# NICTA/revrand

Hardware: AMD Instinct MI355X
Metric: feature-rows/sec (Phi + PhiT Phi + PhiT y) at N=10M D=32 F=4096 (higher is better)
Workload: dtype f32; 1 GPU; RandomRBF nbases=2048 (F=4096), D=32, N=10000000 f32, features + MFMA Gram, rows sharded over 1 GPU(s); rows_per_gpu=10000000, device=(gfx950:sramecc+:xnack-), gram_engine=f32

## Files before the change

### revrand_amd/csrc/rr_mfma_tile.h

```cpp
#pragma once
#include <hip/hip_runtime.h>
#include <cstdint>
#include <cstdlib>

typedef float floatx16 __attribute__((ext_vector_type(16)));
typedef __attribute__((address_space(1))) const void *gptr_t;
typedef __attribute__((address_space(3))) void *lptr_t;

constexpr int GR_TC = 256;
constexpr int GR_KB = 32;
constexpr int GR_LD = 512;
constexpr int GR_THREADS = 512;

typedef float float2v __attribute__((ext_vector_type(2)));

typedef __amdgpu_buffer_rsrc_t rr_rsrc_t;
typedef unsigned rr_u4_t __attribute__((ext_vector_type(4)));
__device__ __forceinline__ rr_rsrc_t rr_make_rsrc(const void *base, unsigned bytes) {
    const uint64_t a = (uint64_t)base;
    const unsigned lo = (unsigned)__builtin_amdgcn_readfirstlane((unsigned)a), hi = (unsigned)__builtin_amdgcn_readfirstlane((unsigned)(a >> 32));
    return __builtin_amdgcn_make_buffer_rsrc((void *)(((uint64_t)hi << 32) | (uint64_t)lo), 0, (int)__builtin_amdgcn_readfirstlane(bytes),
                                             0x00020000);
}

__device__ __forceinline__ void rr_dma_kblock(const float *pa, int64_t lda, const float *pb, int64_t ldb, float *buf, int wave,
                                              unsigned voff) {
    const rr_rsrc_t ra = rr_make_rsrc(pa, 0x7fffffffu), rb = rr_make_rsrc(pb, 0x7fffffffu);
    const unsigned lda4 = (unsigned)lda * 4u, ldb4 = (unsigned)ldb * 4u;
#pragma unroll
    for (int k = 0; k < 4; ++k) {
        const int lr = 4 * wave + k;
        float *dst = buf + lr * GR_LD;
        __builtin_amdgcn_raw_ptr_buffer_load_lds(ra, (lptr_t)dst, 16, voff, (unsigned)lr * lda4, 0, 0);
        __builtin_amdgcn_raw_ptr_buffer_load_lds(rb, (lptr_t)(dst + GR_TC), 16, voff, (unsigned)lr * ldb4, 0, 0);
    }
}
__device__ __forceinline__ int rr_dma_slot(int wave, int spread = 2) {
    return spread == 2 ? (wave < 4 ? wave : ((wave + 2) & 3)) : spread == 1 ? (wave >> 2) : 0;
}
inline int rr_dma_spread_env() {
    const char *e = getenv("RR_DMA_SPREAD");
    return e ? atoi(e) : 2;
}

template <int O0, int O1>
__device__ __forceinline__ float2v lds_read2st64(unsigned addr) {
    float2v r;
    asm volatile("ds_read2st64_b32 %0, %1 offset0:%2 offset1:%3" : "=v"(r) : "v"(addr), "i"(O0), "i"(O1));
    return r;
}
__device__ __forceinline__ void lds_wait() { asm volatile("s_waitcnt lgkmcnt(0)" ::: "memory"); }

struct KOps2 {
    float2v a[4], b[2];
    template <int P>
    __device__ __forceinline__ void load(const unsigned (&abase)[4], const unsigned (&bbase)[2]) {
#pragma unroll
        for (int i = 0; i < 4; ++i) a[i] = lds_read2st64<32 * P, 32 * P + 16>(abase[i]);
#pragma unroll
        for (int j = 0; j < 2; ++j) b[j] = lds_read2st64<32 * P, 32 * P + 16>(bbase[j]);
    }
};

template <int FIRST, int LAST>
__device__ __forceinline__ void gram_mfma(const KOps2 &o, floatx16 (&acc)[4][2]) {
#pragma unroll
    for (int q = FIRST; q < LAST; ++q)
        acc[(q >> 1) & 3][q & 1] = __builtin_amdgcn_mfma_f32_32x32x2f32(o.a[(q >> 1) & 3][q >> 3], o.b[q & 1][q >> 3],
                                                                        acc[(q >> 1) & 3][q & 1], 0, 0, 0);
}

#define RR_PAIR(P, CUR, NXT)                                   \
    lds_wait();                                                \
    __builtin_amdgcn_sched_barrier(0);                         \
    gram_mfma<0, 1>(CUR, acc);                                 \
    __builtin_amdgcn_sched_barrier(0);                         \
    if ((P) + 1 < 8) NXT.template load<((P) + 1) & 7>(abase, bbase); \
    __builtin_amdgcn_sched_barrier(0);                         \
    gram_mfma<1, 16>(CUR, acc);                                \
    __builtin_amdgcn_sched_barrier(0);

__device__ __forceinline__ void gram_consume(unsigned cur, floatx16 (&acc)[4][2], unsigned aoff, unsigned boff) {
    unsigned abase[4], bbase[2];
#pragma unroll
    for (int i = 0; i < 4; ++i) abase[i] = cur + aoff + i * 128;
#pragma unroll
    for (int j = 0; j < 2; ++j) bbase[j] = cur + boff + j * 128;
    KOps2 o0, o1;
    o0.load<0>(abase, bbase);
    RR_PAIR(0, o0, o1) RR_PAIR(1, o1, o0) RR_PAIR(2, o0, o1) RR_PAIR(3, o1, o0)
    RR_PAIR(4, o0, o1) RR_PAIR(5, o1, o0) RR_PAIR(6, o0, o1) RR_PAIR(7, o1, o0)
}

template <typename DMA>
__device__ __forceinline__ void gram_consume_staggered(unsigned cur, floatx16 (&acc)[4][2], unsigned aoff, unsigned boff, int slot,
                                                       DMA dma) {
    unsigned abase[4], bbase[2];
#pragma unroll
    for (int i = 0; i < 4; ++i) abase[i] = cur + aoff + i * 128;
#pragma unroll
    for (int j = 0; j < 2; ++j) bbase[j] = cur + boff + j * 128;
    KOps2 o0, o1;
    if (slot == 0) dma();
    o0.load<0>(abase, bbase);
    RR_PAIR(0, o0, o1)
    if (slot == 1) dma();
    RR_PAIR(1, o1, o0)
    if (slot == 2) dma();
    RR_PAIR(2, o0, o1)
    if (slot == 3) dma();
    RR_PAIR(3, o1, o0)
    RR_PAIR(4, o0, o1) RR_PAIR(5, o1, o0) RR_PAIR(6, o0, o1) RR_PAIR(7, o1, o0)
}
#undef RR_PAIR
```

### revrand_amd/csrc/rr_rff.hip

```cpp
#include "rr_syrk_args.h"
#include <algorithm>
#include <map>
#include <mutex>
#include <type_traits>




__device__ __forceinline__ void sincos_rev(float t, float &s, float &c) {
    const float f = t - __builtin_rintf(t);
    s = __builtin_amdgcn_sinf(f);
    c = __builtin_amdgcn_cosf(f);
}

__device__ __forceinline__ void sincos_rev(double t, double &s, double &c) { rr_sincos_rev_f64(t, s, c); }
typedef double doublex4 __attribute__((ext_vector_type(4)));

template <int DMAX, bool GUARD, typename TX, typename TC>
__device__ __forceinline__ TC project_row(const TX *__restrict__ xr, int d, const TC (&w)[DMAX]) {
    TC z = 0;
#pragma unroll
    for (int i = 0; i < DMAX; ++i) {
        if (!GUARD || i < d) z = fma((TC)xr[i], w[i], z);
    }
// ... 483 lines not shown
    for (int64_t tl = tile0 + wave; tl < tile1; tl += 4) {
        const int64_t r0 = tl * 16;
        double a[KS];
        {
            const int64_t ra = r0 + j;
            const TX *src = X + (ra < N ? ra : 0) * ldx + g * KS;
#pragma unroll
            for (int t = 0; t < KS; ++t) a[t] = (double)src[t];
            if (ra >= N) {
#pragma unroll
                for (int t = 0; t < KS; ++t) a[t] = 0.0;
            }
        }
        const int64_t d0 = N - r0;
        const int lim = (int)(d0 > 16 ? 16 : (d0 < 0 ? 0 : d0));
        double yv[4];
        if (HAS_Y) {
            const int64_t ry = r0 + j;
            double yt = (double)y[ry < N ? ry : N - 1];
            yt = ry < N ? yt : 0.0;
            const int lo = __double2loint(yt), hi = __double2hiint(yt);
#pragma unroll
            for (int e = 0; e < 4; ++e) {
                const int srcl = 4 * (g + 4 * e);
                yv[e] = __hiloint2double(__builtin_amdgcn_ds_bpermute(srcl, hi), __builtin_amdgcn_ds_bpermute(srcl, lo));
            }
        }
        const char *tile_c = (const char *)(P + r0 * ldp + c0);
        const char *tile_s = tile_c + (int64_t)n * (int64_t)sizeof(TO);
        constexpr unsigned ES = sizeof(TO);
        const unsigned lane_off = ES * ((unsigned)g * (unsigned)ldp + (unsigned)j);
#pragma unroll
        for (int cb = 0; cb < CB; ++cb) {
            doublex4 acc = {0.0, 0.0, 0.0, 0.0};
#pragma unroll
            for (int t = 0; t < KS; ++t) acc = __builtin_amdgcn_mfma_f64_16x16x4f64(a[t], bw[cb][t], acc, 0, 0, 0);
            if (c0 + 16 * cb + j < n) {
#pragma unroll
                for (int e = 0; e < 4; ++e) {
                    const int rr = g + 4 * e;
                    const unsigned off = lane_off + ES * 4u * (unsigned)e * (unsigned)ldp;
                    if constexpr (ES == 8) {
                        double sv, cv;
                        rr_sincos_rev_f64(acc[e], sv, cv);
                        cv = rr < lim ? cv * scale : 0.0;
                        sv = rr < lim ? sv * scale : 0.0;
                        asm volatile("global_store_dwordx2 %0, %1, %2 offset:%3 nt" ::"v"(off), "v"(cv), "s"(tile_c), "i"(128 * cb) : "memory");
                        asm volatile("global_store_dwordx2 %0, %1, %2 offset:%3 nt" ::"v"(off), "v"(sv), "s"(tile_s), "i"(128 * cb) : "memory");
                        if (HAS_Y) {
                            bc[cb] = fma(cv, yv[e], bc[cb]);
                            bs[cb] = fma(sv, yv[e], bs[cb]);
                        }
                    } else {
                        const float fr = (float)(acc[e] - rint(acc[e]));
                        const float fs = (float)scale;
                        float cf = __builtin_amdgcn_cosf(fr), sf = __builtin_amdgcn_sinf(fr);
                        cf = rr < lim ? cf * fs : 0.f;
                        sf = rr < lim ? sf * fs : 0.f;
                        asm volatile("global_store_dword %0, %1, %2 offset:%3" RR_NT_ASM ::"v"(off), "v"(cf), "s"(tile_c), "i"(64 * cb) : "memory");
                        asm volatile("global_store_dword %0, %1, %2 offset:%3" RR_NT_ASM ::"v"(off), "v"(sf), "s"(tile_s), "i"(64 * cb) : "memory");
                        if (HAS_Y) {
                            bc[cb] = fma((double)cf, yv[e], bc[cb]);
                            bs[cb] = fma((double)sf, yv[e], bs[cb]);
                        }
                    }
                }
            }
        }
    }
    if (HAS_Y) {
#pragma unroll
        for (int cb = 0; cb < CB; ++cb) {
#pragma unroll
            for (int m = 16; m < 64; m <<= 1) {
                bc[cb] += __hiloint2double(__shfl_xor(__double2hiint(bc[cb]), m, 64), __shfl_xor(__double2loint(bc[cb]), m, 64));
                bs[cb] += __hiloint2double(__shfl_xor(__double2hiint(bs[cb]), m, 64), __shfl_xor(__double2loint(bs[cb]), m, 64));
            }
            const int col = c0 + 16 * cb + j;
            if (g == 0 && col < n) {
                rr_acc_out(bvec, bdet, (int64_t)blockIdx.y * 4 + wave, col, bc[cb]);
                rr_acc_out(bvec, bdet, (int64_t)blockIdx.y * 4 + wave, n + col, bs[cb]);
            }
        }
    }
}

template <typename TX, typename TO>
static bool rr_features_mfma64_launch(rr_basis *b, const TX *X, const TX *y, int64_t m, int64_t mpad, int64_t ldx, TO *P,
                                      int64_t ldp, double *db, double scale) {
    static const bool disabled = getenv("RR_FEATURES_NO_MFMA64") != nullptr;
    if (disabled || b->large || ((ldx * sizeof(TX)) & 15) != 0 || ((uintptr_t)X & 15) != 0 || b->dpad < 8 || m < 1) return false;
    if ((uint64_t)sizeof(TO) * 20u * (uint64_t)ldp >= (1ull << 32)) return false;
    rr_ctx *c = b->ctx;
    const int64_t ntiles = (mpad + 15) / 16;
#define RR_FM64(DM, CBK)                                                                                            \
    do {                                                                                                            \
        const int cgroups = (b->n + 16 * CBK - 1) / (16 * CBK);                                                     \
        int64_t tpb = 128;                                                                                          \
        while (tpb > 4 && cgroups * ((ntiles + tpb - 1) / tpb) < 8 * (int64_t)c->num_cu) tpb >>= 1;                 \
        if ((ntiles + tpb - 1) / tpb > 65535) tpb = (ntiles + 65534) / 65535;                                       \
        const dim3 grid(cgroups, (unsigned)((ntiles + tpb - 1) / tpb));                                             \
        if (y && c->deterministic) {                                                                                \
            void *part = nullptr;                                                                                   \
            const int64_t nslots = (int64_t)grid.y * 4, F2 = 2 * (int64_t)b->n;                                     \
            if (rr_det_scratch(c, (size_t)nslots * F2 * 8, &part) != RR_OK) return false;                           \
            hipLaunchKernelGGL((rr_rff_features_mfma64_kernel<DM, CBK, true, TX, TO>), grid, dim3(256), 0, c->stream, \
                               X, y, m, mpad, ldx, b->dWs64, b->n, b->npad, P, ldp, (double *)part, scale, (int)tpb, F2); \
            if (rr_det_reduce(c, (const double *)part, nslots, F2, F2, db) != RR_OK) return false;                  \
        } else if (y) hipLaunchKernelGGL((rr_rff_features_mfma64_kernel<DM, CBK, true, TX, TO>), grid, dim3(256), 0, c->stream, \
                                  X, y, m, mpad, ldx, b->dWs64, b->n, b->npad, P, ldp, db, scale, (int)tpb);        \
        else hipLaunchKernelGGL((rr_rff_features_mfma64_kernel<DM, CBK, false, TX, TO>), grid, dim3(256), 0, c->stream, \
                                X, y, m, mpad, ldx, b->dWs64, b->n, b->npad, P, ldp, db, scale, (int)tpb);          \
    } while (0)
    switch (b->dpad) {
        case 8: RR_FM64(8, 4); break;
        case 16: RR_FM64(16, 4); break;
        case 32: RR_FM64(32, 4); break;
        case 64: RR_FM64(64, 2); break;
        case 128: RR_FM64(128, 1); break;
        default: return false;
    }
#undef RR_FM64
    return true;
}

template <typename TC>
__global__ void __launch_bounds__(256) rr_zero_padcols_kernel(TC *P, int64_t rows, int64_t ldp, int F) {
    const int w = (int)ldp - F;
    const int64_t i = (int64_t)blockIdx.x * blockDim.x + threadIdx.x;
    if (w > 0 && i < rows * w) P[(i / w) * ldp + F + (i % w)] = TC(0);
}

__global__ void __launch_bounds__(256) rr_zero_padcols_pb_kernel(uintx4 *Pb, int64_t ksteps, int64_t ldp, int F) {
    const int64_t w = (ldp - F) * 4;
    const int64_t i = (int64_t)blockIdx.x * blockDim.x + threadIdx.x;
    if (w > 0 && i < ksteps * w) Pb[(i / w) * ldp * 4 + (int64_t)F * 4 + (i % w)] = uintx4{0u, 0u, 0u, 0u};
}



__device__ __forceinline__ void syrk_dma_tile(const SyrkArgs &p, float *buf, int64_t kb0, int wave, int lane,
                                              int ca, int cb) {
#pragma unroll
    for (int k = 0; k < 4; ++k) {
        const int lr = 4 * wave + k;
        RR_DEV_ASSERT(kb0 + lr < p.rows && ca + GR_TC <= p.ldp && cb + GR_TC <= p.ldp);
        const float *src = p.P + (kb0 + lr) * p.ldp + 4 * lane;
        float *dst = buf + lr * GR_LD;
        __builtin_amdgcn_global_load_lds((gptr_t)(src + ca), (lptr_t)dst, 16, 0, 0);
        __builtin_amdgcn_global_load_lds((gptr_t)(src + cb), (lptr_t)(dst + GR_TC), 16, 0, 0);
    }
}

template <int MODE>
__device__ __forceinline__ void rr_syrk_f32_body(const SyrkArgs &p, float *lds, const unsigned bid) {
    constexpr bool STAG = (MODE & 1) != 0, BUF = (MODE & 2) != 0;

    const int tid = threadIdx.x;
    const int lane = tid & 63;
    const int wave = __builtin_amdgcn_readfirstlane(tid >> 6);

    int tdx = bid % p.ntiles;
    const int ks = bid / p.ntiles;
    if (p.tile_map) tdx = p.tile_map[tdx];
    int ta = 0;
    const int od = p.offdiag_only;
    while (tdx >= p.nb - ta - od) {
        tdx -= p.nb - ta - od;
        ++ta;
    }
    const int tb = ta + tdx + od;
    const bool diag = (ta == tb);
    const int ca = ta * GR_TC, cb = tb * GR_TC;

    const int64_t row_begin = (int64_t)ks * p.rows_per_split;
    int64_t row_end = row_begin + p.rows_per_split;
    if (row_end > p.rows) row_end = p.rows;

    const int wr = wave >> 2, wc_ = wave & 3;
    const unsigned aoff = 4u * ((lane >> 5) * GR_LD + wr * 128 + (lane & 31));
    const unsigned boff = 4u * ((lane >> 5) * GR_LD + GR_TC + wc_ * 64 + (lane & 31));
    const unsigned lds0 = (unsigned)(size_t)(__attribute__((address_space(3))) float *)lds;
    floatx16 acc[4][2];
#pragma unroll
    for (int i = 0; i < 4; ++i)
#pragma unroll
        for (int j = 0; j < 2; ++j)
#pragma unroll
            for (int e = 0; e < 16; ++e) acc[i][j][e] = 0.f;

    const int64_t nkb = (row_end - row_begin) / GR_KB;
    RR_DEV_ASSERT(p.rows % GR_KB == 0 && p.rows_per_split % GR_KB == 0 && tb < p.nb && p.nb * GR_TC <= p.ldp);
    if (BUF && nkb > 0) {
        const unsigned voff = 16u * lane;
        const float *Pa = p.P + row_begin * p.ldp + ca, *Pb = p.P + row_begin * p.ldp + cb;
        rr_dma_kblock(Pa, p.ldp, Pb, p.ldp, lds, wave, voff);
        __syncthreads();
        for (int64_t kb = 0; kb < nkb; ++kb) {
            const int cbuf = (int)(kb & 1);
            float *nxt = lds + (cbuf ^ 1) * (GR_KB * GR_LD);
            const int64_t ro = (kb + 1) * GR_KB * p.ldp;
            if (STAG) {
                gram_consume_staggered(lds0 + cbuf * (4u * GR_KB * GR_LD), acc, aoff, boff, rr_dma_slot(wave, p.spread), [&]() {
                    if (kb + 1 < nkb) rr_dma_kblock(Pa + ro, p.ldp, Pb + ro, p.ldp, nxt, wave, voff);
                });
            } else {
                if (kb + 1 < nkb) rr_dma_kblock(Pa + ro, p.ldp, Pb + ro, p.ldp, nxt, wave, voff);
                gram_consume(lds0 + cbuf * (4u * GR_KB * GR_LD), acc, aoff, boff);
            }
            __syncthreads();
        }
    } else if (nkb > 0) {
        syrk_dma_tile(p, lds, row_begin, wave, lane, ca, cb);
        __syncthreads();
        for (int64_t kb = 0; kb < nkb; ++kb) {
            const int cbuf = (int)(kb & 1);
            float *nxt = lds + (cbuf ^ 1) * (GR_KB * GR_LD);
            if (STAG) {
                const int slot = (wave < 4) ? wave : ((wave + 2) & 3);
                gram_consume_staggered(lds0 + cbuf * (4u * GR_KB * GR_LD), acc, aoff, boff, slot, [&]() {
                    if (kb + 1 < nkb) syrk_dma_tile(p, nxt, row_begin + (kb + 1) * GR_KB, wave, lane, ca, cb);
                });
                __syncthreads();
                continue;
            }
            if (kb + 1 < nkb && !(p.ablate & 1)) syrk_dma_tile(p, nxt, row_begin + (kb + 1) * GR_KB, wave, lane, ca, cb);
            gram_consume(lds0 + cbuf * (4u * GR_KB * GR_LD), acc, aoff, boff);
            if (!(p.ablate & 2)) __syncthreads();
        }
    }

    if (p.ablate & 4) return;
    const int64_t F = p.F;
    const int hi = lane >> 5;
#pragma unroll
    for (int j = 0; j < 2; ++j) {
        const int64_t gc = cb + wc_ * 64 + j * 32 + (lane & 31);
#pragma unroll
        for (int i = 0; i < 4; ++i) {
#pragma unroll
            for (int e = 0; e < 16; ++e) {
                const int64_t gr = ca + wr * 128 + i * 32 + (e & 3) + 8 * (e >> 2) + 4 * hi;
                if (gr <= gc) rr_syrk_out(p, ks, gr, gc, acc[i][j][e]);
            }
        }
    }
    (void)diag;
    (void)F;
}

#define RR_SYRK_KERNEL(NAME, MODE)                                                       \
    __global__ void __launch_bounds__(GR_THREADS, 2) NAME(const SyrkArgs p) {             \
        __shared__ float lds[2 * GR_KB * GR_LD];                                          \
        rr_syrk_f32_body<MODE>(p, lds, blockIdx.x);                                       \
    }
RR_SYRK_KERNEL(rr_syrk_f32_kernel, 3)
RR_SYRK_KERNEL(rr_syrk_f32_flat_kernel, 0)
RR_SYRK_KERNEL(rr_syrk_f32_flatstag_kernel, 1)
RR_SYRK_KERNEL(rr_syrk_f32_buf_kernel, 2)
#undef RR_SYRK_KERNEL

template <int NI>
struct KOpsR {
    float2v a[NI], b[2];
    template <int P>
    __device__ __forceinline__ void load(const unsigned (&abase)[NI], const unsigned (&bbase)[2]) {
#pragma unroll
        for (int i = 0; i < NI; ++i) a[i] = lds_read2st64<32 * P, 32 * P + 16>(abase[i]);
#pragma unroll
        for (int j = 0; j < 2; ++j) b[j] = lds_read2st64<32 * P, 32 * P + 16>(bbase[j]);
    }
};

template <int NI, int FIRST, int LAST>
__device__ __forceinline__ void gram_mfma_r(const KOpsR<NI> &o, floatx16 (&acc)[NI][2]) {
#pragma unroll
    for (int q = FIRST; q < LAST; ++q) {
        constexpr int dummy = 0;
        (void)dummy;
        const int s_ = q / (2 * NI), r_ = q % (2 * NI);
        acc[r_ >> 1][r_ & 1] = __builtin_amdgcn_mfma_f32_32x32x2f32(o.a[r_ >> 1][s_], o.b[r_ & 1][s_], acc[r_ >> 1][r_ & 1], 0, 0, 0);
    }
}

#define RR_PAIRR(P, CUR, NXT)                                  \
    lds_wait();                                                \
    __builtin_amdgcn_sched_barrier(0);                         \
    gram_mfma_r<NI, 0, 1>(CUR, acc);                           \
    __builtin_amdgcn_sched_barrier(0);                         \
    if ((P) + 1 < 8) NXT.template load<((P) + 1) & 7>(abase, bbase); \
    __builtin_amdgcn_sched_barrier(0);                         \
    gram_mfma_r<NI, 1, 4 * NI>(CUR, acc);                      \
    __builtin_amdgcn_sched_barrier(0);

template <int NI>
__device__ __forceinline__ void syrk_ragged_loop(const SyrkArgs &p, float *lds, int wave, int lane, int ca, int cb,
                                                 int64_t row_begin, int64_t nkb, int ks) {
    const int wr = wave >> 2, wc_ = wave & 3;
    const unsigned aoff = 4u * ((lane >> 5) * GR_LD + wr * 128 + (lane & 31));
    const unsigned boff = 4u * ((lane >> 5) * GR_LD + GR_TC + wc_ * 64 + (lane & 31));
    const unsigned lds0 = (unsigned)(size_t)(__attribute__((address_space(3))) float *)lds;
    constexpr int NA = NI > 0 ? NI : 1;
    floatx16 acc[NA][2];
#pragma unroll
    for (int i = 0; i < NA; ++i)
#pragma unroll
        for (int j = 0; j < 2; ++j)
#pragma unroll
            for (int e = 0; e < 16; ++e) acc[i][j][e] = 0.f;
    if (nkb > 0) {
        syrk_dma_tile(p, lds, row_begin, wave, lane, ca, cb);
        __syncthreads();
        for (int64_t kb = 0; kb < nkb; ++kb) {
            const int cbuf = (int)(kb & 1);
            if (kb + 1 < nkb) syrk_dma_tile(p, lds + (cbuf ^ 1) * (GR_KB * GR_LD), row_begin + (kb + 1) * GR_KB, wave, lane, ca, cb);
            if constexpr (NI > 0) {
                const unsigned cur = lds0 + cbuf * (4u * GR_KB * GR_LD);
                unsigned abase[NI], bbase[2];
#pragma unroll
                for (int i = 0; i < NI; ++i) abase[i] = cur + aoff + i * 128;
#pragma unroll
                for (int j = 0; j < 2; ++j) bbase[j] = cur + boff + j * 128;
                KOpsR<NI> o0, o1;
                o0.template load<0>(abase, bbase);
                RR_PAIRR(0, o0, o1) RR_PAIRR(1, o1, o0) RR_PAIRR(2, o0, o1) RR_PAIRR(3, o1, o0)
                RR_PAIRR(4, o0, o1) RR_PAIRR(5, o1, o0) RR_PAIRR(6, o0, o1) RR_PAIRR(7, o1, o0)
            }
            __syncthreads();
        }
    }
    if constexpr (NI > 0) {
        const int hi = lane >> 5;
#pragma unroll
        for (int j = 0; j < 2; ++j) {
            const int64_t grow = cb + wc_ * 64 + j * 32 + (lane & 31);
#pragma unroll
            for (int i = 0; i < NI; ++i) {
#pragma unroll
                for (int e = 0; e < 16; ++e) {
                    const int64_t gcol = ca + wr * 128 + i * 32 + (e & 3) + 8 * (e >> 2) + 4 * hi;
                    rr_syrk_out(p, ks, grow, gcol, acc[i][j][e]);
                }
            }
        }
    }
}
#undef RR_PAIRR

__global__ void __launch_bounds__(GR_THREADS, 2)
rr_syrk_f32_ragged_kernel(const SyrkArgs p) {
    __shared__ float lds[2 * GR_KB * GR_LD];
    const int lane = threadIdx.x & 63;
    const int wave = __builtin_amdgcn_readfirstlane(threadIdx.x >> 6);
    const int last = p.nb - 1;
    const int ta = blockIdx.x % last;
    const int ks = blockIdx.x / last;
    const int ca = last * GR_TC;
    const int cb = ta * GR_TC;
    const int64_t row_begin = (int64_t)ks * p.rows_per_split;
    int64_t row_end = row_begin + p.rows_per_split;
    if (row_end > p.rows) row_end = p.rows;
    const int64_t nkb = (row_end - row_begin) / GR_KB;
    RR_DEV_ASSERT(p.rows % GR_KB == 0 && p.rows_per_split % GR_KB == 0 && p.nb * GR_TC == p.ldp && p.F > ca);
    const int w = p.F + (p.bcol ? 1 : 0) - ca;
    int ni = (w - (wave >> 2) * 128 + 31) / 32;
    ni = ni < 0 ? 0 : (ni > 4 ? 4 : ni);
    switch (ni) {
        case 0: syrk_ragged_loop<0>(p, lds, wave, lane, ca, cb, row_begin, nkb, ks); break;
        case 1: syrk_ragged_loop<1>(p, lds, wave, lane, ca, cb, row_begin, nkb, ks); break;
        case 2: syrk_ragged_loop<2>(p, lds, wave, lane, ca, cb, row_begin, nkb, ks); break;
        case 3: syrk_ragged_loop<3>(p, lds, wave, lane, ca, cb, row_begin, nkb, ks); break;
        default: syrk_ragged_loop<4>(p, lds, wave, lane, ca, cb, row_begin, nkb, ks); break;
    }
}

__constant__ unsigned char RR_DIAG_I[8][5] = {{0, 0, 0, 0, 0}, {1, 1, 1, 1, 1}, {2, 2, 2, 2, 2}, {3, 3, 3, 3, 3},
                                              {0, 0, 0, 7, 0}, {1, 1, 6, 6, 1}, {2, 5, 5, 5, 2}, {4, 4, 4, 4, 4}};
__constant__ unsigned char RR_DIAG_J[8][5] = {{0, 1, 2, 3, 4}, {1, 2, 3, 4, 5}, {2, 3, 4, 5, 6}, {3, 4, 5, 6, 7},
                                              {5, 6, 7, 7, 5}, {6, 7, 6, 7, 6}, {7, 5, 6, 7, 7}, {4, 5, 6, 7, 4}};

template <int NB>
struct KOpsD {
    float2v a[NB], b[NB];
    template <int P>
    __device__ __forceinline__ void load(const unsigned (&abase)[NB], const unsigned (&bbase)[NB]) {
#pragma unroll
        for (int e = 0; e < NB; ++e) a[e] = lds_read2st64<16 * P, 16 * P + 8>(abase[e]);
#pragma unroll
        for (int e = 0; e < NB; ++e) b[e] = lds_read2st64<16 * P, 16 * P + 8>(bbase[e]);
    }
};

template <int NB, int FIRST, int LAST>
__device__ __forceinline__ void gram_mfma_d(const KOpsD<NB> &o, floatx16 (&acc)[NB]) {
#pragma unroll
    for (int q = FIRST; q < LAST; ++q)
        acc[q % NB] = __builtin_amdgcn_mfma_f32_32x32x2f32(o.a[q % NB][q / NB], o.b[q % NB][q / NB], acc[q % NB], 0, 0, 0);
}

#define RR_PAIRD(P, CUR, NXT)                                  \
    lds_wait();                                                \
    __builtin_amdgcn_sched_barrier(0);                         \
    gram_mfma_d<NB, 0, 1>(CUR, acc);                           \
    __builtin_amdgcn_sched_barrier(0);                         \
    if ((P) + 1 < 8) NXT.template load<((P) + 1) & 7>(abase, bbase); \
    __builtin_amdgcn_sched_barrier(0);                         \
    gram_mfma_d<NB, 1, 2 * NB>(CUR, acc);                      \
    __builtin_amdgcn_sched_barrier(0);

template <int NB>
__device__ __forceinline__ void syrk_diag_body(const SyrkArgs &p, float *lds, int wave, int lane) {
    const int ta = blockIdx.x % p.nb;
    const int ks = blockIdx.x / p.nb;
// ... 1359 lines not shown
            if (d <= 0 || (double)(next() >> 11) / 9007199254740992.0 < exp(-(double)d / temp)) {
                add(x, t1, -1); add(y, t2, -1); add(x, t2, 1); add(y, t1, 1);
                part[t1] = y; part[t2] = x;
                cur += d;
                if (cur < best) { best = cur; best_part = part; }
            }
        }
        part = best_part;
    }
    std::vector<int> fill(nxcd, 0);
    for (int t = 0; t < ntiles; ++t) map[(size_t)fill[part[t]]++ * nxcd + part[t]] = t;
}


int rr_launch_syrk_f32(rr_ctx *c, const float *P, int64_t rows, int64_t ldp, int F, double *dG, hipEvent_t mid,
                       double *bcol = nullptr) {
    if (c->gram_engine != 0) {
        RR_REQUIRE(bcol == nullptr, "gram: the rider column needs the f32 engine");
        RR_REQUIRE(!c->deterministic, "gram: deterministic mode (rr_set_deterministic) needs the f32 engine, not a split 16-bit one");
        return rr_launch_syrk_bf16(c, c->gram_engine, P, nullptr, rows, ldp, F, dG, mid);
    }
    RR_REQUIRE(bcol == nullptr || F < ldp, "gram: no pad column for the rider");
    static const bool small_off = getenv("RR_SYRK_SMALL") != nullptr && atoi(getenv("RR_SYRK_SMALL")) == 0;
    const int64_t big_tiles = (ldp / GR_TC) * (ldp / GR_TC + 1) / 2;
    if (!small_off && ldp <= 1024 && big_tiles * ((rows + 1023) / 1024) < c->num_cu && rows % GS_KB == 0 && !getenv("RR_GRAM_ABLATE")) {
        const int nbs = (int)(ldp / GS_TC), nt = nbs * (nbs + 1) / 2;
        int64_t ns = std::max<int64_t>((2 * c->num_cu + nt - 1) / nt, (rows + 32767) / 32768);
        ns = std::min<int64_t>(ns, std::max<int64_t>(rows / 128, 1));
        const int64_t rps_s = ((rows + ns - 1) / ns + GS_KB - 1) / GS_KB * GS_KB;
        ns = (rows + rps_s - 1) / rps_s;
        SyrkArgs a;
        a.P = P; a.rows = rows; a.ldp = ldp; a.F = F; a.nb = nbs; a.ntiles = nt; a.rows_per_split = rps_s; a.G = dG;
        a.bcol = bcol; a.tile_map = nullptr; a.offdiag_only = 0; a.ablate = 0;
        if (c->deterministic) {
            void *slabs = nullptr;
            int rc = rr_det_scratch(c, (size_t)ns * (size_t)ldp * (size_t)ldp * sizeof(float), &slabs);
            if (rc != RR_OK) return rc;
            a.part = (float *)slabs;
            a.part_stride = ldp * ldp;
        }
        hipLaunchKernelGGL(rr_syrk_f32_small_kernel, dim3((unsigned)(ns * nt)), dim3(GS_THREADS), 0, c->stream, a);
        if (mid) RR_CHECK_HIP(hipEventRecord(mid, c->stream));
        if (a.part)
            hipLaunchKernelGGL(rr_syrk_det_reduce_kernel<float>, dim3((unsigned)((F + 1 + 255) / 256), (unsigned)F), dim3(256), 0,
                               c->stream, a.part, a.part_stride, ldp, F, (int)ns, dG, bcol);
        RR_CHECK_HIP(hipGetLastError());
        return RR_OK;
    }
    const int nb_all = (int)(ldp / GR_TC);
    const int od = (nb_all >= 2 && !getenv("RR_SYRK_NO_DIAG_KERNEL")) ? 1 : 0;
    const int w_last = F + (bcol ? 1 : 0) - GR_TC * (nb_all - 1);
    const int rg = (od && nb_all >= 3 && w_last <= 192 && !getenv("RR_SYRK_NO_RAGGED_KERNEL")) ? 1 : 0;
    const int nb = nb_all - rg;
    const int ntiles = od ? nb * (nb - 1) / 2 : nb * (nb + 1) / 2;
    const int nxcd = 8;
    const bool use_map = (ntiles % nxcd == 0) && !getenv("RR_GRAM_NO_TILE_MAP");
    if (use_map && c->tile_map_nb != nb * 2 + od) {
        std::vector<int> map;
        rr_build_tile_map(nb, od, nxcd, map);
        if (c->tile_map) (void)hipFree(c->tile_map);
        c->tile_map = nullptr;
        RR_CHECK_HIP(hipMalloc((void **)&c->tile_map, map.size() * sizeof(int)));
        RR_CHECK_HIP(hipMemcpy(c->tile_map, map.data(), map.size() * sizeof(int), hipMemcpyHostToDevice));
        c->tile_map_nb = nb * 2 + od;
    }
    const int64_t total_tiles = (int64_t)nb_all * (nb_all + 1) / 2;
    auto gcd64 = [](int64_t x, int64_t y) { while (y) { const int64_t u = x % y; x = y; y = u; } return x; };
    const int64_t min_splits = (rows + 32767) / 32768;
    auto rows_per = [&](int64_t ns) { return ((rows + ns - 1) / ns + GR_KB - 1) / GR_KB * GR_KB; };
    const int64_t unit = ntiles > 0 ? c->num_cu / gcd64(c->num_cu, ntiles) : 1;
    int64_t nsplit = (min_splits + unit - 1) / unit * unit;
    auto floor_rows = [&](int64_t tiles_per_split) {
        return tiles_per_split * ((rows + 1023) / 1024) < c->num_cu ? (int64_t)256 : (int64_t)1024;
    };
    auto small_split = [&](int64_t tiles_per_split) {
        const int64_t fr = floor_rows(tiles_per_split);
        if (fr == 1024) return (rows + 1023) / 1024;
        const int64_t want = (c->num_cu + tiles_per_split - 1) / std::max<int64_t>(tiles_per_split, 1);
        return std::min((rows + fr - 1) / fr, std::max((rows + 1023) / 1024, want));
    };
    if (rows / nsplit < 1024) {
        nsplit = small_split(std::max(ntiles, 1));
        static const bool no_search = getenv("RR_SYRK_SPLIT_SEARCH") != nullptr && atoi(getenv("RR_SYRK_SPLIT_SEARCH")) == 0;
        if (ntiles > 0 && !no_search) {
            double best_cost = 1e300;
            int64_t best_ns = nsplit;
            const int64_t ns_hi = std::max<int64_t>(rows / 256, 1), ns_lo = std::max<int64_t>(rows / 32768, 1);
            for (int64_t ns = ns_lo; ns <= ns_hi && ns <= ns_lo + 4096; ++ns) {
                const int64_t rp = rows_per(ns), n2 = (rows + rp - 1) / rp;
                const int64_t rounds = ((int64_t)ntiles * n2 + c->num_cu - 1) / c->num_cu;
                const double cost = (double)rounds * ((double)rp + 96.0);
                if (cost < best_cost - 1e-9) {
                    best_cost = cost;
                    best_ns = n2;
                }
            }
            nsplit = best_ns;
        }
    }
    if (nsplit < 1) nsplit = 1;
    int64_t rps = rows_per(nsplit);
    int64_t nsplit_d = nsplit, rps_d = rps;
    if (od) {
        double best = -1.0;
        for (int64_t ns = min_splits; ns < min_splits + 96; ++ns) {
            if (rows / ns < floor_rows(nb_all) && ns > 1) break;
            const int64_t wg = ns * nb_all, rounds = (wg + c->num_cu - 1) / c->num_cu;
            const double eff = (double)wg / (double)(rounds * c->num_cu);
            if (eff > best + 1e-9) {
                best = eff;
                nsplit_d = ns;
            }
        }
        rps_d = rows_per(nsplit_d);
        if (rows % 64 == 0 && getenv("RR_SYRK_DIAG_KB") != nullptr && atoi(getenv("RR_SYRK_DIAG_KB")) == 64)
            rps_d = (rps_d + 63) / 64 * 64;
    }
    int64_t nsplit_r = nsplit, rps_r = rps;
    if (rg) {
        double best = -1.0;
        for (int64_t ns = min_splits; ns < min_splits + 96; ++ns) {
            if (rows / ns < floor_rows(nb_all - 1) && ns > 1) break;
            const int64_t wg = ns * (nb_all - 1), rounds = (wg + c->num_cu - 1) / c->num_cu;
            const double eff = (double)wg / (double)(rounds * c->num_cu);
            if (eff > best + 1e-9) {
                best = eff;
                nsplit_r = ns;
            }
        }
        rps_r = rows_per(nsplit_r);
    }
    const char *renv = getenv("RR_GRAM_ROWS_PER_SPLIT");
    if (renv && atoll(renv) >= GR_KB) rps = rps_d = rps_r = (atoll(renv) / GR_KB) * GR_KB;
    if (c->deterministic) rps_d = rps_r = rps;
    nsplit = (rows + rps - 1) / rps;
    nsplit_d = (rows + rps_d - 1) / rps_d;
    nsplit_r = (rows + rps_r - 1) / rps_r;
    RR_REQUIRE(nsplit * total_tiles < (int64_t)1 << 31 && nsplit_d * nb_all < (int64_t)1 << 31 &&
                   nsplit_r * nb_all < (int64_t)1 << 31, "gram: grid too large");
    SyrkArgs a;
    a.P = P; a.rows = rows; a.ldp = ldp; a.F = F; a.nb = nb; a.ntiles = ntiles; a.rows_per_split = rps; a.G = dG;
    a.bcol = bcol;
    a.tile_map = use_map ? c->tile_map : nullptr;
    a.offdiag_only = od;
    a.ablate = getenv("RR_GRAM_ABLATE") ? atoi(getenv("RR_GRAM_ABLATE")) : 0;
    a.spread = rr_dma_spread_env();
    if (c->deterministic) {
        void *slabs = nullptr;
        int rc = rr_det_scratch(c, (size_t)nsplit * (size_t)ldp * (size_t)ldp * sizeof(float), &slabs);
        if (rc != RR_OK) return rc;
        a.part = (float *)slabs;
        a.part_stride = ldp * ldp;
    }
    static const int syrk_mode = getenv("RR_SYRK_STAGGER") ? atoi(getenv("RR_SYRK_STAGGER")) : 3;
    static const bool merge_diag = getenv("RR_SYRK_MERGE_DIAG") != nullptr && atoi(getenv("RR_SYRK_MERGE_DIAG")) != 0;
    if (merge_diag && od && !rg && ntiles > 0 && syrk_mode == 3 && !a.ablate && !getenv("RR_SYRK_NO_DIAG16")) {
        SyrkArgs ad = a;
        ad.nb = nb_all;
        ad.rows_per_split = rps_d;
        const unsigned n_off = (unsigned)(nsplit * ntiles);
        hipLaunchKernelGGL(rr_syrk_f32_merged_kernel, dim3(n_off + (unsigned)(nsplit_d * nb_all)), dim3(GR_THREADS), 0, c->stream, a, ad, n_off);
        if (mid) RR_CHECK_HIP(hipEventRecord(mid, c->stream));
        if (a.part)
            hipLaunchKernelGGL(rr_syrk_det_reduce_kernel<float>, dim3((unsigned)((F + 1 + 255) / 256), (unsigned)F), dim3(256), 0,
                               c->stream, a.part, a.part_stride, ldp, F, (int)nsplit, dG, bcol);
        RR_CHECK_HIP(hipGetLastError());
        return RR_OK;
    }
    if (ntiles > 0) {
        if (syrk_mode == 1 && !a.ablate)
            hipLaunchKernelGGL(rr_syrk_f32_flatstag_kernel, dim3((unsigned)(nsplit * ntiles)), dim3(GR_THREADS), 0, c->stream, a);
        else if (syrk_mode == 2 && !a.ablate)
            hipLaunchKernelGGL(rr_syrk_f32_buf_kernel, dim3((unsigned)(nsplit * ntiles)), dim3(GR_THREADS), 0, c->stream, a);
        else if (syrk_mode == 0 || a.ablate)
            hipLaunchKernelGGL(rr_syrk_f32_flat_kernel, dim3((unsigned)(nsplit * ntiles)), dim3(GR_THREADS), 0, c->stream, a);
        else
            hipLaunchKernelGGL(rr_syrk_f32_kernel, dim3((unsigned)(nsplit * ntiles)), dim3(GR_THREADS), 0, c->stream, a);
    }
    if (rg) {
        SyrkArgs ar = a;
        ar.nb = nb_all;
        ar.rows_per_split = rps_r;
        hipLaunchKernelGGL(rr_syrk_f32_ragged_kernel, dim3((unsigned)(nsplit_r * (nb_all - 1))), dim3(GR_THREADS), 0, c->stream, ar);
    }
    if (mid) RR_CHECK_HIP(hipEventRecord(mid, c->stream));
    if (od) {
        SyrkArgs ad = a;
        ad.nb = nb_all;
        ad.rows_per_split = rps_d;
        static const bool no_diag16 = getenv("RR_SYRK_NO_DIAG16") != nullptr;
        static const bool kb64 = getenv("RR_SYRK_DIAG_KB") != nullptr && atoi(getenv("RR_SYRK_DIAG_KB")) == 64;
        if (no_diag16)
            hipLaunchKernelGGL(rr_syrk_f32_diag_kernel, dim3((unsigned)(nsplit_d * nb_all)), dim3(GR_THREADS), 0, c->stream, ad);
        else if (kb64 && rows % 64 == 0 && ad.rows_per_split % 64 == 0)
            hipLaunchKernelGGL(rr_syrk_f32_diag16_kernel<64>, dim3((unsigned)(nsplit_d * nb_all)), dim3(GR_THREADS), 0, c->stream, ad);
        else
            hipLaunchKernelGGL(rr_syrk_f32_diag16_kernel<32>, dim3((unsigned)(nsplit_d * nb_all)), dim3(GR_THREADS), 0, c->stream, ad);
    }
    if (a.part)
        hipLaunchKernelGGL(rr_syrk_det_reduce_kernel<float>, dim3((unsigned)((F + 1 + 255) / 256), (unsigned)F), dim3(256), 0,
                           c->stream, a.part, a.part_stride, ldp, F, (int)nsplit, dG, bcol);
    RR_CHECK_HIP(hipGetLastError());
    return RR_OK;
}

int rr_launch_syrk_f64(rr_ctx *c, const double *P, int64_t rows, int64_t ldp, int F, double *dG, int lower_tri = 0) {
    const int nb = (int)(ldp / G64_TC);
    const int od = (nb >= 2 && !getenv("RR_SYRK_NO_DIAG_KERNEL")) ? 1 : 0;
    const int ntiles = od ? nb * (nb - 1) / 2 : nb * (nb + 1) / 2;
    const int64_t slots = (int64_t)c->num_cu * 2;
    int64_t g = slots, t = ntiles;
    while (t) { const int64_t u = g % t; g = t; t = u; }
    const int64_t unit = slots / g;
    static const bool no_fine = getenv("RR_SYRK64_FINE_SPLIT") != nullptr && atoi(getenv("RR_SYRK64_FINE_SPLIT")) == 0;
    const int64_t min_rows = (lower_tri && rows == ldp && rows <= 2048 && !no_fine) ? 128 : 512;
    int64_t nsplit = unit;
    if (rows / nsplit < 2048) nsplit = (slots * 4 + ntiles - 1) / ntiles;
    if (rows / nsplit < min_rows) nsplit = (rows + min_rows - 1) / min_rows;
    if (nsplit < 1) nsplit = 1;
    const int64_t rps = ((rows + nsplit - 1) / nsplit + G64_KB - 1) / G64_KB * G64_KB;
    nsplit = (rows + rps - 1) / rps;
    RR_REQUIRE(nsplit * ntiles < (int64_t)1 << 31, "gram: grid too large");
    Syrk64Args a;
    a.P = P; a.rows = rows; a.ldp = ldp; a.F = F; a.nb = nb; a.ntiles = ntiles; a.rows_per_split = rps; a.G = dG;
    a.offdiag_only = od;
    static const bool no_tri = getenv("RR_SYRK64_TRI") != nullptr && atoi(getenv("RR_SYRK64_TRI")) == 0;
    a.lower_tri = lower_tri && !no_tri && rows == ldp ? 1 : 0;
    if (c->deterministic) {
        void *slabs = nullptr;
        int rc = rr_det_scratch(c, (size_t)nsplit * (size_t)ldp * (size_t)ldp * sizeof(double), &slabs);
        if (rc != RR_OK) return rc;
        a.part = (double *)slabs;
        a.part_stride = ldp * ldp;
    }
    if (ntiles > 0)
        hipLaunchKernelGGL(rr_syrk_f64_kernel, dim3((unsigned)(nsplit * ntiles)), dim3(G64_THREADS), 0, c->stream, a);
    if (od) {
        const int64_t dslots = (int64_t)c->num_cu * 4;
        int64_t best_ns = 1;
        double best = -1.0;
        for (int64_t ns = 1; ns <= 4 * dslots / nb + 1; ++ns) {
            if (rows / ns < min_rows && ns > 1) break;
            const int64_t wg = ns * nb, rounds = (wg + dslots - 1) / dslots;
            const double eff = (double)wg / (double)(rounds * dslots);
            if (eff > best + 1e-9) {
                best = eff;
                best_ns = ns;
            }
        }
        Syrk64Args ad = a;
        ad.rows_per_split = ((rows + best_ns - 1) / best_ns + G64_KB - 1) / G64_KB * G64_KB;
        if (c->deterministic) ad.rows_per_split = rps;
        const int64_t nsd = (rows + ad.rows_per_split - 1) / ad.rows_per_split;
        hipLaunchKernelGGL(rr_syrk_f64_diag_kernel, dim3((unsigned)(nsd * nb)), dim3(G64_THREADS), 0, c->stream, ad);
    }
    if (a.part)
        hipLaunchKernelGGL(rr_syrk_det_reduce_kernel<double>, dim3((unsigned)((F + 255) / 256), (unsigned)F), dim3(256), 0,
                           c->stream, a.part, a.part_stride, ldp, F, (int)nsplit, dG, (double *)nullptr);
    RR_CHECK_HIP(hipGetLastError());
    return RR_OK;
}

int rr_launch_gemm_tn_f64(rr_ctx *c, const double *A, int64_t lda, const double *B, int64_t ldb, double *D, int64_t ldd,
                          int64_t K, int64_t M, int64_t N, int subtract, int upper_only) {
    Gemm64Args g;
    g.A = A; g.B = B; g.D = D; g.lda = lda; g.ldb = ldb; g.ldd = ldd; g.K = (int)K; g.ntb = (int)(N / G64_TC);
    g.subtract = subtract;
    g.upper_only = upper_only;
    static const bool no_k128 = getenv("RR_GEMM64_K128") != nullptr && atoi(getenv("RR_GEMM64_K128")) == 0;
    if (!no_k128 && K == 128 && M == 128 && N % 32 == 0 && (upper_only == 0 || (upper_only == 1 && N == 128))) {
        hipLaunchKernelGGL(rr_gemm_tn_f64_k128_kernel, dim3((unsigned)(N / 32)), dim3(G64_THREADS), 0, c->stream, g);
        RR_CHECK_HIP(hipGetLastError());
        return RR_OK;
    }
    hipLaunchKernelGGL(rr_gemm_tn_f64_kernel, dim3((unsigned)((M / G64_TC) * g.ntb)), dim3(G64_THREADS), 0, c->stream, g);
    RR_CHECK_HIP(hipGetLastError());
    return RR_OK;
}

template <typename TX, typename TC>
static int launch_gram(rr_basis *b, const void *dX, const void *dy, int64_t N, int64_t ldx, double *dG,
                       double *db) {
    rr_ctx *c = b->ctx;
    constexpr bool F32 = sizeof(TC) == 4;
    constexpr int TCOLS = F32 ? GR_TC : G64_TC;
    constexpr int KB = F32 ? GR_KB : G64_KB;
    const int F = 2 * b->n;
    const int64_t ldp = ((int64_t)F + TCOLS - 1) / TCOLS * TCOLS;
    const TC scale = (TC)(1.0 / sqrt((double)b->n));
    const TC *Ws = F32 ? (const TC *)b->dWs32 : (const TC *)b->dWs64;
    int64_t chunk = (int64_t)(((size_t)32 << 30) / ((size_t)ldp * sizeof(TC)));
    const char *cenv = getenv("RR_GRAM_CHUNK_ROWS");
    if (cenv && atoll(cenv) >= KB) chunk = atoll(cenv);
    else if (N > chunk) {
        const int64_t nchunks = (N + chunk - 1) / chunk;
        chunk = (N + nchunks - 1) / nchunks;
    }
    if (chunk > N) chunk = N;
    RR_REQUIRE(!(F32 && c->deterministic && c->gram_engine != 0),
               "gram: deterministic mode (rr_set_deterministic) needs the f32 engine, not a split 16-bit one");
    const bool fused_pb = F32 && !b->phase64 && c->gram_engine != 0 && rr_features_mfma_ok<TX>(b, (const TX *)dX, N, ldx);
    const int KBR = fused_pb ? 64 : KB;
    chunk = (chunk + KBR - 1) / KBR * KBR;
    static const bool overlap_on = getenv("RR_GRAM_OVERLAP") != nullptr && atoi(getenv("RR_GRAM_OVERLAP")) != 0;
    const bool overlap = N > chunk && overlap_on && !c->deterministic;
    const int nbuf = overlap ? 2 : 1;
    int rc = ensure_zbuf(b, (size_t)nbuf * (size_t)chunk * ldp * sizeof(TC));
    if (rc != RR_OK) return rc;
    TC *P = (TC *)b->zbuf;
    if (overlap && !c->stream2) {
        RR_CHECK_HIP(hipStreamCreateWithFlags(&c->stream2, hipStreamNonBlocking));
        RR_CHECK_HIP(hipEventCreateWithFlags(&c->ev_fork, hipEventDisableTiming));
    }
    hipStream_t fstream = overlap ? c->stream2 : c->stream;
    const hipStream_t main_stream = c->stream;
    if (fused_pb && ldp > F) {
        const int64_t cnt = (nbuf * chunk / 16) * (ldp - F) * 4;
        hipLaunchKernelGGL(rr_zero_padcols_pb_kernel, dim3((unsigned)((cnt + 255) / 256)), dim3(256), 0, c->stream,
                           (uintx4 *)P, nbuf * chunk / 16, ldp, F);
        RR_CHECK_HIP(hipGetLastError());
    } else if (ldp > F) {
        const int64_t cnt = nbuf * chunk * (ldp - F);
        hipLaunchKernelGGL(rr_zero_padcols_kernel<TC>, dim3((unsigned)((cnt + 255) / 256)), dim3(256), 0, c->stream,
                           P, nbuf * chunk, ldp, F);
        RR_CHECK_HIP(hipGetLastError());
    }

    TC *const Pbase = P;
// ... 810 lines not shown
```

Before: 8.528 million feature-rows/s.

## Add skewed half-slab ring pipeline for f32 SYRK Gram kernel and make it default

Adds a new SYRK mode that splits each 32-row k-block into 16-row half slabs held in a 5-entry LDS ring. The two wave groups run half a block apart: waves 0-3 start immediately and waves 4-7 follow one half-step behind. Each wave DMAs its half slab two ring slots ahead, and operand reads for the next half are preloaded across half boundaries. The aim is to stop all eight waves from stalling at the same barrier and to keep MFMA issue busy while loads are in flight. The LDS footprint goes from 64 to 80 rows per block, which could reduce occupancy, and the ring indexing adds correctness risk.

Result: no change. 8.564 million feature-rows/s (median of 6 runs) (+0.4%).

```diff
diff --git a/revrand_amd/csrc/rr_mfma_tile.h b/revrand_amd/csrc/rr_mfma_tile.h
--- a/revrand_amd/csrc/rr_mfma_tile.h
+++ b/revrand_amd/csrc/rr_mfma_tile.h
@@ -113,3 +113,56 @@
     RR_PAIR(4, o0, o1) RR_PAIR(5, o1, o0) RR_PAIR(6, o0, o1) RR_PAIR(7, o1, o0)
 }
 #undef RR_PAIR
+
+constexpr int GR_HS = 16;
+constexpr int GR_RING = 5;
+constexpr unsigned GR_HS_BYTES = 4u * GR_HS * GR_LD;
+
+__device__ __forceinline__ unsigned rr_ring(unsigned g) { return g >= (unsigned)GR_RING ? g - (unsigned)GR_RING : g; }
+
+__device__ __forceinline__ void rr_dma_kblock_half(const float *pa, int64_t lda, const float *pb, int64_t ldb, float *half, int wave,
+                                                   unsigned voff) {
+    const rr_rsrc_t ra = rr_make_rsrc(pa, 0x7fffffffu), rb = rr_make_rsrc(pb, 0x7fffffffu);
+    const unsigned lda4 = (unsigned)lda * 4u, ldb4 = (unsigned)ldb * 4u;
+#pragma unroll
+    for (int k = 0; k < 4; ++k) {
+        const int lr = 4 * wave + k;
+        float *dst = half + (4 * (wave & 3) + k) * GR_LD;
+        __builtin_amdgcn_raw_ptr_buffer_load_lds(ra, (lptr_t)dst, 16, voff, (unsigned)lr * lda4, 0, 0);
+        __builtin_amdgcn_raw_ptr_buffer_load_lds(rb, (lptr_t)(dst + GR_TC), 16, voff, (unsigned)lr * ldb4, 0, 0);
+    }
+}
+
+__device__ __forceinline__ void gram_half_bases(unsigned (&abase)[4], unsigned (&bbase)[2], unsigned hs, unsigned aoff, unsigned boff) {
+#pragma unroll
+    for (int i = 0; i < 4; ++i) abase[i] = aoff + (hs + i * 128);
+#pragma unroll
+    for (int j = 0; j < 2; ++j) bbase[j] = boff + (hs + j * 128);
+}
+
+#define RR_HPAIR(CUR, READS)                                   \
+    lds_wait();                                                \
+    __builtin_amdgcn_sched_barrier(0);                         \
+    gram_mfma<0, 1>(CUR, acc);                                 \
+    __builtin_amdgcn_sched_barrier(0);                         \
+    READS;                                                     \
+    __builtin_amdgcn_sched_barrier(0);                         \
+    gram_mfma<1, 16>(CUR, acc);                                \
+    __builtin_amdgcn_sched_barrier(0);
+template <bool WITH_DMA, bool PRELOAD, typename DMA>
+__device__ __forceinline__ void gram_consume_half(KOps2 &o0, KOps2 &o1, unsigned (&abase)[4], unsigned (&bbase)[2],
+                                                  floatx16 (&acc)[4][2], unsigned nxt, unsigned aoff, unsigned boff, int slot,
+                                                  DMA dma) {
+    if (WITH_DMA && slot == 0) dma();
+    RR_HPAIR(o0, o1.template load<1>(abase, bbase))
+    if (WITH_DMA && slot == 1) dma();
+    RR_HPAIR(o1, o0.template load<2>(abase, bbase))
+    if (WITH_DMA && slot == 2) dma();
+    RR_HPAIR(o0, o1.template load<3>(abase, bbase))
+    if (WITH_DMA && slot == 3) dma();
+    RR_HPAIR(o1, if (PRELOAD) {
+        gram_half_bases(abase, bbase, nxt, aoff, boff);
+        o0.template load<0>(abase, bbase);
+    })
+}
+#undef RR_HPAIR
diff --git a/revrand_amd/csrc/rr_rff.hip b/revrand_amd/csrc/rr_rff.hip
--- a/revrand_amd/csrc/rr_rff.hip
+++ b/revrand_amd/csrc/rr_rff.hip
@@ -659,9 +659,57 @@
     }
 }
 
+template <bool LATE>
+__device__ __forceinline__ void syrk_skew_loop(const SyrkArgs &p, float *lds, const unsigned lds0, floatx16 (&acc)[4][2], const float *Pa,
+                                               const float *Pb, const int64_t nkb, const int wave, const unsigned voff, const unsigned aoff,
+                                               const unsigned boff) {
+    const int slot = rr_dma_slot(wave, p.spread);
+    unsigned abase[4], bbase[2];
+    KOps2 o0, o1;
+    unsigned q = 0;
+    int64_t kb = 0;
+    auto dma = [&]() {
+        if (kb + 1 < nkb) {
+            const unsigned dst = rr_ring(q + 2u + (unsigned)(wave >> 2));
+            RR_DEV_ASSERT(dst < (unsigned)GR_RING && dst != q && dst != rr_ring(q + 1u) && dst != rr_ring(q + 4u));
+            RR_DEV_ASSERT((dst * GR_HS + 4u * (wave & 3) + 4u) * GR_LD * 4u <= GR_RING * GR_HS_BYTES);
+            RR_DEV_ASSERT((kb + 1) * GR_KB + 4 * wave + 3 < p.rows);
+            const int64_t ro = (kb + 1) * GR_KB * p.ldp;
+            rr_dma_kblock_half(Pa + ro, p.ldp, Pb + ro, p.ldp, lds + dst * (GR_HS * GR_LD), wave, voff);
+        }
+    };
+    if (!LATE) {
+        for (; kb < nkb; ++kb) {
+            RR_DEV_ASSERT(q == (unsigned)((2 * kb) % GR_RING));
+            gram_half_bases(abase, bbase, lds0 + q * GR_HS_BYTES, aoff, boff);
+            o0.load<0>(abase, bbase);
+            gram_consume_half<true, true>(o0, o1, abase, bbase, acc, lds0 + rr_ring(q + 1u) * GR_HS_BYTES, aoff, boff, slot, dma);
+            gram_consume_half<false, false>(o0, o1, abase, bbase, acc, 0u, aoff, boff, slot, dma);
+            q = rr_ring(q + 2u);
+            __syncthreads();
+        }
+    } else {
+        gram_half_bases(abase, bbase, lds0, aoff, boff);
+        o0.load<0>(abase, bbase);
+        gram_consume_half<true, true>(o0, o1, abase, bbase, acc, lds0 + GR_HS_BYTES, aoff, boff, slot, dma);
+        lds_wait();
+        __syncthreads();
+        q = 2u;
+        for (kb = 1; kb < nkb; ++kb) {
+            RR_DEV_ASSERT(q == (unsigned)((2 * kb) % GR_RING));
+            gram_consume_half<true, true>(o0, o1, abase, bbase, acc, lds0 + q * GR_HS_BYTES, aoff, boff, slot, dma);
+            gram_consume_half<false, true>(o0, o1, abase, bbase, acc, lds0 + rr_ring(q + 1u) * GR_HS_BYTES, aoff, boff, slot, dma);
+            q = rr_ring(q + 2u);
+            lds_wait();
+            __syncthreads();
+        }
+        gram_consume_half<false, false>(o0, o1, abase, bbase, acc, 0u, aoff, boff, slot, dma);
+    }
+}
+
 template <int MODE>
 __device__ __forceinline__ void rr_syrk_f32_body(const SyrkArgs &p, float *lds, const unsigned bid) {
-    constexpr bool STAG = (MODE & 1) != 0, BUF = (MODE & 2) != 0;
+    constexpr bool SKEW = MODE == 4, STAG = !SKEW && (MODE & 1) != 0, BUF = !SKEW && (MODE & 2) != 0;
 
     const int tid = threadIdx.x;
     const int lane = tid & 63;
@@ -698,7 +746,14 @@
 
     const int64_t nkb = (row_end - row_begin) / GR_KB;
     RR_DEV_ASSERT(p.rows % GR_KB == 0 && p.rows_per_split % GR_KB == 0 && tb < p.nb && p.nb * GR_TC <= p.ldp);
-    if (BUF && nkb > 0) {
+    if (SKEW && nkb > 0) {
+        const unsigned voff = 16u * lane;
+        const float *Pa = p.P + row_begin * p.ldp + ca, *Pb = p.P + row_begin * p.ldp + cb;
+        rr_dma_kblock_half(Pa, p.ldp, Pb, p.ldp, lds + (wave >> 2) * (GR_HS * GR_LD), wave, voff);
+        __syncthreads();
+        if (wave < 4) syrk_skew_loop<false>(p, lds, lds0, acc, Pa, Pb, nkb, wave, voff, aoff, boff);
+        else syrk_skew_loop<true>(p, lds, lds0, acc, Pa, Pb, nkb, wave, voff, aoff, boff);
+    } else if (BUF && nkb > 0) {
         const unsigned voff = 16u * lane;
         const float *Pa = p.P + row_begin * p.ldp + ca, *Pb = p.P + row_begin * p.ldp + cb;
         rr_dma_kblock(Pa, p.ldp, Pb, p.ldp, lds, wave, voff);
@@ -761,11 +816,15 @@
         __shared__ float lds[2 * GR_KB * GR_LD];                                          \
         rr_syrk_f32_body<MODE>(p, lds, blockIdx.x);                                       \
     }
-RR_SYRK_KERNEL(rr_syrk_f32_kernel, 3)
+RR_SYRK_KERNEL(rr_syrk_f32_lockstep_kernel, 3)
 RR_SYRK_KERNEL(rr_syrk_f32_flat_kernel, 0)
 RR_SYRK_KERNEL(rr_syrk_f32_flatstag_kernel, 1)
 RR_SYRK_KERNEL(rr_syrk_f32_buf_kernel, 2)
 #undef RR_SYRK_KERNEL
+__global__ void __launch_bounds__(GR_THREADS, 2) rr_syrk_f32_kernel(const SyrkArgs p) {
+    __shared__ float lds[GR_RING * GR_HS * GR_LD];
+    rr_syrk_f32_body<4>(p, lds, blockIdx.x);
+}
 
 template <int NI>
 struct KOpsR {
@@ -2431,9 +2490,9 @@
         a.part = (float *)slabs;
         a.part_stride = ldp * ldp;
     }
-    static const int syrk_mode = getenv("RR_SYRK_STAGGER") ? atoi(getenv("RR_SYRK_STAGGER")) : 3;
+    static const int syrk_mode = getenv("RR_SYRK_STAGGER") ? atoi(getenv("RR_SYRK_STAGGER")) : 4;
     static const bool merge_diag = getenv("RR_SYRK_MERGE_DIAG") != nullptr && atoi(getenv("RR_SYRK_MERGE_DIAG")) != 0;
-    if (merge_diag && od && !rg && ntiles > 0 && syrk_mode == 3 && !a.ablate && !getenv("RR_SYRK_NO_DIAG16")) {
+    if (merge_diag && od && !rg && ntiles > 0 && syrk_mode >= 3 && !a.ablate && !getenv("RR_SYRK_NO_DIAG16")) {
         SyrkArgs ad = a;
         ad.nb = nb_all;
         ad.rows_per_split = rps_d;
@@ -2453,6 +2512,8 @@
             hipLaunchKernelGGL(rr_syrk_f32_buf_kernel, dim3((unsigned)(nsplit * ntiles)), dim3(GR_THREADS), 0, c->stream, a);
         else if (syrk_mode == 0 || a.ablate)
             hipLaunchKernelGGL(rr_syrk_f32_flat_kernel, dim3((unsigned)(nsplit * ntiles)), dim3(GR_THREADS), 0, c->stream, a);
+        else if (syrk_mode == 3)
+            hipLaunchKernelGGL(rr_syrk_f32_lockstep_kernel, dim3((unsigned)(nsplit * ntiles)), dim3(GR_THREADS), 0, c->stream, a);
         else
             hipLaunchKernelGGL(rr_syrk_f32_kernel, dim3((unsigned)(nsplit * ntiles)), dim3(GR_THREADS), 0, c->stream, a);
     }
```
